# alebeck/jax-raft

Hardware: AMD Instinct MI355X
Metric: image-pairs/sec + Sintel-clean EPE, raft_large 32 iters at 1/2/4/8 MI355X (higher is better)
Workload: dtype bf16

## Files before the change

### csrc/kernels/conv_halo.hip

```cpp
#include "halo.h"

namespace {

template <int P>
JR_DEVICE constexpr int key_x(int key) { return P == 8 ? (key >> 1) & 7 : key & 15; }

JR_DEVICE int lane_px(int rho) {
  return rho < 4 ? rho : rho < 12 ? rho + 12 : rho < 16 ? rho - 8 : rho < 20 ? rho + 8 : rho < 28 ? rho - 12 : rho;
}

template <int CIN>
constexpr int pitch_of() { return CIN <= 64 ? 8 : CIN <= 128 ? 16 : 32; }

template <int CIN, int WCO, int WPX, int TN, bool INN>
constexpr int halo_min_blocks() {
  return TN > 2 ? 1 : CIN <= 64 ? 4 : CIN <= 96 ? (INN ? 3 : 1) : !INN ? 1 : WCO * WPX == 1 ? 4 : WCO * WPX <= 4 ? 2 : 1;
}

template <int CIN, int WCO, int WPX, int TN, int TR, int TC, bool INN, int KS = 3>
__global__ __launch_bounds__(64 * WCO * WPX, (halo_min_blocks<CIN, WCO, WPX, TN, INN>()))
void conv_halo_kernel(const ConvHaloParams p) {
  constexpr int NT = 64 * WCO * WPX;
  constexpr int P = pitch_of<CIN>();
  constexpr int CC = CIN / 8;
  constexpr int SPT = CIN / 16;
  constexpr int S = KS * KS * SPT;
  constexpr int PAD = KS / 2;
  constexpr bool WIDE = TN >= 4 && WCO * WPX > 4;
  constexpr bool MANY = WCO * WPX >= 12;
  constexpr int PD = S >= 16 ? (WCO * WPX >= 16 ? 4 : (WIDE || MANY || CIN <= 96) ? 8 : 16) : S;
  constexpr int FW = TC + KS - 1;
  constexpr int NFP = (TR + KS - 1) * FW;
  constexpr int RB = P * 16;
  static_assert(TR * TC <= 32 * WPX * TN && (TC == 16 || TC == 8), "tile");
  extern __shared__ __attribute__((aligned(16))) bf16 lds[];
  char* const lds_b = (char*)lds;
  const int tid = threadIdx.x, lane = tid & 63, wave = tid >> 6;
  const int rho = lane & 31, hh = lane >> 5;
  const int wc = wave % WCO, wp = wave / WCO;

  const int per_img = p.tiles_y * p.tiles_x;
  const int n = blockIdx.x / per_img;
  const int rem = blockIdx.x - n * per_img;
  const int ty = rem / p.tiles_x, tx = rem - ty * p.tiles_x;
  const int y0 = ty * TR, x0 = tx * TC;
// ... 284 lines not shown
```

### csrc/kernels/halo.h

```cpp
#pragma once
#include "conv_igemm.h"

namespace {

constexpr unsigned HOOB = 0x80000000u;
constexpr int FPITCH = 256;
constexpr int RPITCH = 128;

JR_DEVICE int f_off(int row, int chunk) { return row * FPITCH + (((chunk & 16) | ((chunk ^ row) & 15)) << 3); }
JR_DEVICE int r_off(int row, int chunk) { return row * RPITCH + (((chunk ^ row) & 15) << 3); }

JR_DEVICE u32x4 bload(__amdgpu_buffer_rsrc_t r, unsigned off) {
  return __builtin_bit_cast(u32x4, __builtin_amdgcn_raw_buffer_load_b128(r, off, 0, 0));
}

template <int NB, int S, int PD, typename LA, typename RB>
JR_DEVICE void pipe_gemm(f32x16 (&acc)[NB], bf16x8 (&ring)[PD], LA&& loadA, RB&& readB) {
#pragma unroll
  for (int b = 0; b < NB; ++b)
#pragma unroll
    for (int k = 0; k < 16; ++k) acc[b][k] = 0.f;
  bf16x8 bcur[NB], bnxt[NB];
#pragma unroll
  for (int b = 0; b < NB; ++b) bcur[b] = readB(0, b);
#pragma unroll
  for (int s = 0; s < S; ++s) {
    const bf16x8 a = ring[s % PD];
    if (s + PD < S) ring[s % PD] = loadA(s + PD);
    if (s + 1 < S) {
#pragma unroll
      for (int b = 0; b < NB; ++b) bnxt[b] = readB(s + 1, b);
    }
#pragma unroll
    for (int b = 0; b < NB; ++b) acc[b] = __builtin_amdgcn_mfma_f32_32x32x16_bf16(a, bcur[b], acc[b], 0, 0, 0);
#pragma unroll
    for (int b = 0; b < NB; ++b) bcur[b] = bnxt[b];
    __builtin_amdgcn_sched_group_barrier(0x100, NB, 0);
    __builtin_amdgcn_sched_group_barrier(0x020, 1, 0);
    __builtin_amdgcn_sched_group_barrier(0x008, NB, 0);
    asm volatile("" ::: "memory");
    __builtin_amdgcn_sched_barrier(0);
  }
}

}
```

### csrc/kernels/kernels.h

```cpp
#pragma once
#include <hip/hip_runtime.h>
#include <stdint.h>

extern "C" {

enum ConvEpi : int {
  EPI_STD = 0,
  EPI_GRU_A = 1,
  EPI_GRU_B = 2,
  EPI_BWD = 5,
  EPI_TAPS = 6,
};

struct BwdSeg {
  int mode;
  const void* gin; int gin_cs, gin_coff, gin_bf16;
  const void* mask; int mask_cs, mask_coff;
  int valid;
  void* out; int out_cs, out_coff, out_f32;
};

struct ConvParams {
  const void* x;
  int N, H, W;
// ... 149 lines not shown
int jr_unsup_loss_blocks(long P);
int jr_unsup_loss(const float* pred, const float* img1, const float* img2, const float* mask, const float* prm,
                  float* part, int B, int H, int W, int N, hipStream_t stream);
int jr_unsup_loss_bwd(const float* pred, const float* img1, const float* img2, const float* mask, const float* prm,
                      const float* scale, float* grad, int B, int H, int W, int N, hipStream_t stream);
long jr_census_tiles(int B, int H, int W);
int jr_census_gray(const float* img1, const float* img2, float* gray, int B, int H, int W, hipStream_t stream);
int jr_census_loss(const float* pred, const float* gray, const float* mask, const float* prm, float* part, float* coef,
                   int B, int H, int W, int N, hipStream_t stream);
int jr_census_loss_bwd(const float* pred, const float* gray, const float* coef, const float* scale, float* grad, int B,
                       int H, int W, int N, int add, hipStream_t stream);
#define JR_RANGE_MAX_PIXELS (1L << 23)
int jr_range_splat(const float* flow_fw, const float* flow_bw, int* acc, int B, int H, int W, hipStream_t stream);
int jr_range_visible(const float* flow_fw, const float* flow_bw, const int* acc, float* vis, int B, int H, int W,
                     int T, hipStream_t stream);
int jr_crop_resize(const float* x, const float* prm, float* out, int B, int H, int W, int C, int c, hipStream_t stream);
int jr_selfsup_loss_blocks(long P);
int jr_selfsup_loss(const float* pred, const float* target, const float* weight, const float* prm, float* part, int N,
                    int B, int H, int W, int Btot, int B0, hipStream_t stream);
int jr_selfsup_loss_bwd(const float* pred, const float* target, const float* weight, const float* prm, const float* scale,
                        float* grad, int N, int B, int H, int W, int Btot, int B0, hipStream_t stream);
struct Conv1x1Args {
  const void* x; int xcs, kvalid, kpad; const void* wpk; const float* bias; int act;
  void* y; int ycs, ycoff, cout, M;
};
int jr_flowin_dual(const void* x, int x_cstride, int N, int H, int W, int PH, int PW, const void* w,
                   const float* fbias, int cout, int relu, void* y, int y_cstride, int y_coff, int mode,
                   const void* feat, int feat_cstride, int feat_coff, const void* wpk, const float* cbias, float alpha,
                   const float* flow, float* out, const void* out_slot, long out_off, const Conv1x1Args* c1,
                   hipStream_t stream);
int jr_conv_direct(const void* x, int x_cstride, int N, int H, int W, int cin, int KH, int KW, int PH, int PW,
                   const void* w, const float* bias, int cout, int relu, void* y, int y_cstride, int y_coff,
                   hipStream_t stream);
int jr_copy_channels(const void* src, int s_cstride, int s_coff, void* dst, int d_cstride, int d_coff,
                     int M, int C, hipStream_t stream);

struct ConvF32Params {
  const float* x; int N, H, W, x_cs, x_coff, cin4;
  int KH, KW, SH, SW, PH, PW, OH, OW, M;
  const float* w; int K, cout;
  const float* bias; float alpha; int act, split;
  float* y; int y_cs, y_coff;
  float* y2; int y2_cs, y2_coff;
  const float* res; int res_cs, res_coff, res_post;
  float* h32; float* zbuf; int hidden;
  const float* bmap; int bmap_cs, bmap_coff;
  int ksplit; float* part;
};
int jr_conv_f32(const ConvF32Params* p, int epi, hipStream_t stream);
int jr_channel_stats_f32(const float* x, int N, int HW, int C, float* stats, float* partial, hipStream_t stream);
int jr_norm_act_f32(const float* x, const float* sx, int mode_x, const float* res, const float* sr, int mode_r,
                    float* y, int N, int HW, int C, float eps, int relu, hipStream_t stream);
int jr_prep_images_f32(const float* img1, const float* img2, int B, int H, int W, float* out, hipStream_t stream);
int jr_copy_channels_f32(const float* src, int s_cstride, int s_coff, float* dst, int d_cstride, int d_coff, int M,
                         int C, hipStream_t stream);
int jr_upsample_convex_f32(const float* mask, int mask_cstride, const float* flow, int B, int h, int w, float* out,
                           const void* out_slot, long out_off, hipStream_t stream);
int jr_corr_pool_f32(const float* src, long M, int hl, int wl, float* dst, hipStream_t stream);
int jr_corr_lookup_f32(const float* const* levels, int num_levels, int B, int h, int w, int nq, int radius,
                       const float* coords, float* out, int out_cstride, hipStream_t stream);
int jr_flow_update_f32(const float* delta, int dcs, int N, int h, int w, float* coords, float* flow32, float* hx,
                       int hx_cs, int hx_off, float* qx, int qx_cs, int qx_off, float* flow4, hipStream_t stream);

struct GruFusedParams {
  const void* hx; int hx_cs;
  const void* wa; const void* wb;
// ... 73 lines not shown
```

### csrc/runtime/binding.cpp

```cpp
#include <torch/custom_class.h>
#include <torch/library.h>
#include <ATen/ATen.h>
#include <c10/core/DeviceGuard.h>
#include <c10/hip/HIPStream.h>
#include <hip/hip_runtime.h>

#include <algorithm>
#include <array>
#include <functional>
#include <string>
#include <vector>

#include "../kernels/kernels.h"
#include "plan.h"

namespace jr {

using TList = c10::List<c10::optional<at::Tensor>>;
using IList = std::vector<int64_t>;

static inline at::Tensor opt(const TList& t, size_t i) {
  if (i >= t.size()) return at::Tensor();
  c10::optional<at::Tensor> v = t.get(i);
  return v.has_value() ? *v : at::Tensor();
// ... 787 lines not shown
              "taps_gemm: packed weights (pack_taps)");
  TORCH_CHECK(cs(taps) >= 24 && cs(taps) % 4 == 0 && taps.numel() >= M * cs(taps) &&
                  reinterpret_cast<uintptr_t>(taps.data_ptr()) % 16 == 0,
              "taps_gemm: taps [M][>=24], 16-byte rows");
  keep.push_back(fm); keep.push_back(wpk); keep.push_back(taps);
  const void* fp = fm.data_ptr();
  const void* wp = wpk.data_ptr();
  float* tp = taps.data_ptr<float>();
  const int fcs = cs(fm), tcs = cs(taps);
  return [=](hipStream_t s, int) { return jr_taps_gemm(fp, fcs, fcoff, K, wp, tp, tcs, (int)M, s); };
}

static Launch make_conv_direct(const TList& t, const IList& i, std::vector<at::Tensor>& keep) {
  at::Tensor x = opt(t, 0), w = opt(t, 1), bias = opt(t, 2), y = opt(t, 3);
  check_bf16(x, "x"); check_bf16(w, "w"); check_f32(bias, "bias"); check_bf16(y, "y");
  const int N = (int)i[0], H = (int)i[1], W = (int)i[2], cin = (int)i[3], KH = (int)i[4], KW = (int)i[5];
  const int PH = (int)i[6], PW = (int)i[7], cout = (int)i[8], relu = (int)i[9], y_coff = (int)i[10];
  const int64_t M = (int64_t)N * H * W;
  TORCH_CHECK(cs(x) >= cin && x.numel() >= M * cs(x), "conv_direct: x [N*H*W][>=cin]");
  const int kwp = KW <= 4 ? 4 : 8, nkc = (KH * kwp * 2 + 31) / 32;
  TORCH_CHECK(cin == 2 && w.numel() == (int64_t)cout * nkc * 32 && bias.numel() >= cout, "conv_direct: w / bias");
  TORCH_CHECK(y.numel() >= M * cs(y) && y_coff + cout <= cs(y), "conv_direct: y");
  for (auto& v : {x, w, bias, y}) keep.push_back(v);
  const void* xp = x.data_ptr();
  const void* wp = w.data_ptr();
  const float* bp = bias.data_ptr<float>();
  void* yp = y.data_ptr();
  const int xcs = cs(x), ycs = cs(y);
  return [=](hipStream_t s, int) {
    return jr_conv_direct(xp, xcs, N, H, W, cin, KH, KW, PH, PW, wp, bp, cout, relu, yp, ycs, y_coff, s);
  };
}

static Launch make_flowin_dual(const TList& t, const IList& i, double alpha, std::vector<at::Tensor>& keep) {
  Launch conv = make_conv_direct(t, IList(i.begin(), i.begin() + 11), keep);
  TORCH_CHECK((i.size() == 15 || i.size() == 21) && i[4] == 7 && i[5] == 7,
              "flowin_dual: expected 15 (+6) ints, a 7x7 flow conv");
  const bool has_c1 = i.size() == 21;
  Conv1x1Args c1a{};
  if (has_c1) {
    TORCH_CHECK(i[11] == 2 && i[17] == 352, "flowin_dual: the 1x1 conv part needs mode 2 and K padded to 352");
    TList t1;
    for (size_t k = 10; k < 14; ++k) t1.push_back(c10::optional<at::Tensor>(opt(t, k)));
    (void)make_conv1x1(t1, IList(i.begin() + 15, i.end()), keep);
    at::Tensor x1 = opt(t, 10), w1 = opt(t, 11), b1 = opt(t, 12), y1 = opt(t, 13);
    c1a = Conv1x1Args{x1.data_ptr(), (int)cs(x1), (int)i[16], (int)i[17], w1.data_ptr(), b1.data_ptr<float>(),
                      (int)i[19], y1.data_ptr(), (int)cs(y1), (int)i[20], (int)i[18], (int)i[15]};
  }
  at::Tensor x = opt(t, 0), w = opt(t, 1), bias = opt(t, 2), y = opt(t, 3), flow = opt(t, 4), out = opt(t, 5),
             slot = opt(t, 6), feat = opt(t, 7), wpk = opt(t, 8), cb = opt(t, 9);
  const int N = (int)i[0], H = (int)i[1], W = (int)i[2], PH = (int)i[6], PW = (int)i[7], cout = (int)i[8];
  const int relu = (int)i[9], y_coff = (int)i[10], mode = (int)i[11], fcoff = (int)i[14];
  const int64_t stride = i[12], slot_off = i[13];
  check_f32(flow, "flow32");
  TORCH_CHECK(mode == 1 || mode == 2, "flowin_dual: mode 1 (bilinear) or 2 (convex head)");
  TORCH_CHECK(flow.numel() >= (int64_t)N * H * W * 2, "flowin_dual: flow [M][2]");
  TORCH_CHECK(!slot.defined() || (slot.is_cuda() && slot.scalar_type() == at::kLong && slot.numel() == 1),
              "flowin_dual: out_slot must be one device int64");
  const int64_t cap = check_flow_out(out, N, H, W);
  TORCH_CHECK(stride >= 0 && stride % 8 == 0, "flowin_dual: iteration stride");
  int fcs = 0;
  if (mode == 2) {
    check_bf16(feat, "feat"); check_bf16(wpk, "wpk"); check_f32(cb, "cbias");
    fcs = cs(feat);
    TORCH_CHECK(fcs % 8 == 0 && fcoff % 8 == 0 && fcoff >= 0 && fcoff + 256 <= fcs &&
                    feat.numel() >= (int64_t)N * H * W * fcs && reinterpret_cast<uintptr_t>(feat.data_ptr()) % 16 == 0,
// ... 1332 lines not shown

static const std::vector<OpRow>& op_table() {
  static const std::vector<OpRow> rows = {
      row_tia("conv", "alpha", 22, 29, make_conv_fwd),
      row_tia("corr", "scale", 5, 7, make_corr),
      row_ti("lookup", 5, 9, make_lookup, 1),
      row_ti("feat_pool", 5, 5, make_feat_pool),
      row_ti("lookup_od", 6, 8, make_lookup_od, 1),
      row_ti("upsample_convex", 4, 4, make_upsample_convex),
      row_tia("convex_head", "alpha", 5, 7, make_convex_head),
      row_ti("upsample_bilinear", 4, 5, make_upsample_bilinear),
      row_ti("stats", 3, 3, make_stats),
      row_ti("stats_final", 3, 3, make_stats_final),
      row_tia("norm_act", "eps", 6, 6, make_norm_act),
      row_ti("prep", 3, 8, make_prep),
      row_ti("init_coords", 3, 3, make_init_coords),
      row_ti("init_flow", 5, 5, make_init_flow_bf16),
      row_ti("init_flow_f32", 5, 5, make_init_flow_f32),
      row_ti("forward_project", 4, 4, make_forward_project),
      row_ti("fb_check", 7, 9, make_fb_check),
      row_ti("warp_frames", 8, 10, make_warp_frames),
      row_t("memset", make_memset),
      row_t("copy", make_copy),
      row_ti("copy_channels", 4, 4, make_copy_channels),
      row_ti("sum_iters", 2, 2, make_sum_iters),
      row_ti("im2col", 11, 11, make_im2col),
      row_ti("flow_taps", 5, 5, make_flow_taps),
      row_ti("taps_gemm", 3, 3, make_taps_gemm),
      row_ti("gru_fused", 4, 5, make_gru_fused),
      row_ti("gru_fused_me", 4, 4, make_gru_fused_me),
      row_ti("gru_halo", 9, 9, make_gru_halo),
      row_ti("conv1x1", 6, 6, make_conv1x1),
      row_ti("conv_direct", 11, 11, make_conv_direct),
      row_tia("flowin_dual", "alpha", 15, 21, make_flowin_dual),
      row_tia("upsample_convex_bwd", "alpha", 3, 3, make_upsample_convex_bwd),
      row_ti("upsample_bilinear_bwd", 3, 3, make_upsample_bilinear_bwd),
      row_ti("flow_gather_bwd", 3, 3, make_flow_gather_bwd),
      row_ti("lookup_bwd", 5, 6, make_lookup_bwd),
      row_tia("norm_bwd", "eps", 5, 5, make_norm_bwd),
      row_ti("pack", 2, 2, make_pack),
      row_ti("wgrad", 16, 16, make_wgrad),
      row_ti("bn_table", 2, 2, make_bn_table),
      row_ti("augment_sums", 3, 3, make_augment_sums_of<JR_AUGMENT_DENSE>),
      row_ti("augment", 5, 5, make_augment_gather_of<JR_AUGMENT_DENSE>),
      row_ti("augment_sparse_sums", 3, 3, make_augment_sums_of<JR_AUGMENT_SPARSE>),
      row_ti("augment_sparse", 5, 5, make_augment_gather_of<JR_AUGMENT_SPARSE>),
      row_ti("augment_mixed_sums", 2, 2, make_augment_sums_of<JR_AUGMENT_MIXED>),
      row_ti("augment_mixed", 4, 4, make_augment_gather_of<JR_AUGMENT_MIXED>),
      row_ti("flow_metrics", 6, 6, make_flow_metrics),
      row_ti("unsup_loss", 4, 4, make_unsup_loss),
      row_ti("unsup_loss_bwd", 4, 4, make_unsup_loss_bwd),
      row_ti("census_gray", 3, 3, make_census_gray),
      row_ti("census_loss", 4, 4, make_census_loss),
      row_ti("census_loss_bwd", 5, 5, make_census_loss_bwd),
      row_ti("range_splat", 3, 3, make_range_splat),
      row_ti("range_visible", 4, 4, make_range_visible),
      row_ti("crop_resize", 5, 5, make_crop_resize),
      row_ti("selfsup_loss", 6, 6, make_selfsup_loss),
      row_ti("selfsup_loss_bwd", 6, 6, make_selfsup_loss_bwd),
      row_tia("conv_f32", "alpha", 22, 22, make_conv_f32),
      row_ti("stats_f32", 3, 3, make_stats_f32),
      row_tia("norm_act_f32", "eps", 6, 6, make_norm_act_f32),
      row_ti("prep_f32", 3, 3, make_prep_f32),
      row_ti("copy_channels_f32", 4, 4, make_copy_channels_f32),
      row_ti("upsample_convex_f32", 4, 5, make_upsample_convex_f32),
      row_ti("corr_pool_f32", 3, 3, make_corr_pool_f32),
// ... 108 lines not shown
```

### jax_raft_amd/_build.py

```python
from __future__ import annotations

import concurrent.futures as cf
import os
import subprocess
import sys
import sysconfig
from pathlib import Path

PKG_DIR = Path(__file__).resolve().parent
REPO = PKG_DIR.parent
CSRC = REPO / "csrc"
BUILD = REPO / "build" / "native"
SO_PATH = PKG_DIR / "_C.so"
ARCH = os.environ.get("JR_OFFLOAD_ARCH") or "gfx950"
HIPCC = os.environ.get("HIPCC", "/opt/rocm/bin/hipcc")
CXX = os.environ.get("CXX", "g++")

KERNEL_SOURCES = [
    CSRC / "kernels" / "conv_igemm.hip",
    CSRC / "kernels" / "conv_fam_r.hip",
    CSRC / "kernels" / "conv_fam_rw.hip",
    CSRC / "kernels" / "conv_fam_p.hip",
    CSRC / "kernels" / "conv_fam_m32.hip",
    CSRC / "kernels" / "conv_fam_d2.hip",
    CSRC / "kernels" / "conv_fam_g.hip",
    CSRC / "kernels" / "corr.hip",
    CSRC / "kernels" / "corr_pyr.hip",
    CSRC / "kernels" / "corr_od.hip",
    CSRC / "kernels" / "elementwise.hip",
    CSRC / "kernels" / "conv_f32.hip",
    CSRC / "kernels" / "f32.hip",
    CSRC / "kernels" / "flowhead.hip",
    CSRC / "kernels" / "conv_direct.hip",
    CSRC / "kernels" / "train.hip",
    CSRC / "kernels" / "wgrad.hip",
    CSRC / "kernels" / "convex_head.hip",
    CSRC / "kernels" / "conv1x1.hip",
    CSRC / "kernels" / "gru_fused.hip",
    CSRC / "kernels" / "gru_halo.hip",
    CSRC / "kernels" / "conv_halo.hip",
    CSRC / "kernels" / "bgemm.hip",
    CSRC / "kernels" / "merged.hip",
    CSRC / "kernels" / "conv_fam_grp.hip",
    CSRC / "kernels" / "warm.hip",
    CSRC / "kernels" / "fbcheck.hip",
    CSRC / "kernels" / "framewarp.hip",
    CSRC / "kernels" / "augment.hip",
    CSRC / "kernels" / "metrics.hip",
    CSRC / "kernels" / "unsup.hip",
    CSRC / "kernels" / "census.hip",
    CSRC / "kernels" / "occlusion.hip",
    CSRC / "kernels" / "selfsup.hip",
]
HOST_SOURCES = [CSRC / "runtime" / "binding.cpp", CSRC / "runtime" / "png.cpp"]
HEADERS = sorted(CSRC.rglob("*.h"))


def _torch_paths():
    import torch
    from torch.utils import cpp_extension

    inc = cpp_extension.include_paths(device_type="cuda")
    lib = os.path.join(os.path.dirname(torch.__file__), "lib")
    abi = int(torch._C._GLIBCXX_USE_CXX11_ABI)
    return inc, lib, abi

# ... 70 lines not shown
```

### jax_raft_amd/ops/native.py

```python
from __future__ import annotations

import math
import threading
from dataclasses import dataclass
from pathlib import Path
from typing import List, Optional, Sequence, Tuple

import torch

from .. import knobs
from .._build import SO_PATH as _DEFAULT_SO

SO_PATH = Path(knobs.get("JR_NATIVE_SO")).resolve() if knobs.get("JR_NATIVE_SO") else _DEFAULT_SO

_lock = threading.Lock()
_loaded = False
_load_error: Optional[BaseException] = None

ACT_NONE, ACT_RELU, ACT_SIGMOID, ACT_TANH, ACT_SPLIT_TANH_RELU = 0, 1, 2, 3, 4
EPI_STD, EPI_GRU_A, EPI_GRU_B = 0, 1, 2
EPI_BWD, EPI_TAPS = 5, 6
TAPS_CFGS = (34, 22, 35, 38)
CFG_TILES = {0: (128, 128), 1: (64, 128), 2: (128, 64), 3: (16, 256), 4: (64, 64), 5: (16, 64)}
CFG_TILES.update({6: (128, 128), 7: (64, 128), 8: (128, 64), 9: (128, 256), 10: (64, 64), 11: (256, 128)})
CFG_TILES.update({12: (128, 128), 13: (64, 128), 14: (128, 64), 15: (64, 64)})
CFG_TILES.update({16: (256, 128), 17: (128, 256)})
CFG_TILES.update({18: (128, 128), 19: (128, 128), 20: (256, 128)})
CFG_TILES.update({21: (128, 128), 22: (256, 128), 23: (128, 64), 24: (64, 128)})
CFG_TILES.update({25: (256, 128), 26: (128, 256), 27: (128, 128), 28: (64, 256)})
CFG_TILES.update({33: (128, 128), 34: (256, 128)})
CFG_TILES.update({35: (256, 128), 36: (128, 128), 37: (128, 128), 38: (256, 128), 39: (256, 128), 40: (128, 256),
                  41: (64, 128), 42: (256, 128), 43: (256, 128)})
TUNE_CFGS = (0, 1, 2, 3, 4, 5, 12, 13, 14, 15, 18, 19, 20, 21, 22, 23, 24, 25, 26, 27, 28, 33, 34,
             35, 38)
NUM_CUS = 256
GROUPED_CFGS = frozenset((2, 4, 5, 23, 24, 12, 14, 15))


def gru_fused_tiles(N: int, H: int, W: int, vertical: int) -> int:
    if not vertical:
        return N * H if 1 <= W <= 128 else 0
    J = 2 if 2 * H <= 128 and W % 2 == 0 else 1
    return N * (W // J) if 1 <= H and J * H <= 128 and J * (H + 4) <= 136 and W % J == 0 else 0


def _m32_chan(r: torch.Tensor) -> torch.Tensor:
    return 16 * ((r >> 2) & 1) + (r & 3) + 4 * (r >> 3)


def pack_gru_halo(kernel: torch.Tensor, cin_pad: int, out: Optional[torch.Tensor] = None) -> torch.Tensor:
    kh, kw, cin, cout = kernel.shape
    assert cout % 32 == 0 and cin <= cin_pad and cin_pad % 16 == 0, (kernel.shape, cin_pad)
    dev = kernel.device
    k = torch.zeros(kh * kw, cin_pad, cout, dtype=torch.float32, device=dev)
    k[:, :cin] = kernel.detach().float().reshape(kh * kw, cin, cout)
    k = k.reshape(kh * kw * cin_pad, cout)
    ks = kh * kw * cin_pad // 16
    blk = torch.arange(cout // 32, device=dev).view(-1, 1, 1, 1)
    s = torch.arange(ks, device=dev).view(1, -1, 1, 1)
    l = torch.arange(64, device=dev).view(1, 1, 64, 1)
    j = torch.arange(8, device=dev).view(1, 1, 1, 8)
    kk = (16 * s + 8 * (l >> 5) + j).expand(cout // 32, ks, 64, 8)
    co = (32 * blk + _m32_chan(l & 31)).expand(cout // 32, ks, 64, 8)
    w = k[kk, co].to(torch.bfloat16).contiguous()
    if out is not None:
        assert out.shape == w.shape and out.dtype == torch.bfloat16
        out.copy_(w)
        return out
    return w


GRU_HALO_BLOCKS = {(128, 0): ((1, 1), (2, 1), (2, 2), (3, 2), (3, 3), (5, 4)), (96, 1): ((2, 1), (2, 2), (3, 2))}


def gru_halo_lds(hd: int, mode: int, TR: int, TC: int, nb1: int, nb2: int) -> int:
    f_rows = TC + 8 if mode == 0 else (TR + 4) * (TC + 4)
# ... 305 lines not shown
    lane = torch.arange(64, device=dev).view(1, 1, 1, 64, 1)
    j = torch.arange(8, device=dev).view(1, 1, 1, 1, 8)
    o = 16 * t + lane % 16
    c = 64 * g + 16 * (lane // 16) + 8 * s + j
    return wt[o.expand(4, 2, 2, 64, 8), c.expand(4, 2, 2, 64, 8)].to(torch.bfloat16).contiguous()


CONV1X1_KPADS = (128, 256, 352, 384)


def pack_conv1x1(kernel: torch.Tensor, kpad: int) -> torch.Tensor:
    _, _, K, N = kernel.shape
    assert N % 64 == 0 and K <= kpad and kpad % 32 == 0, (kernel.shape, kpad)
    w = torch.zeros(kpad, N, dtype=torch.float32, device=kernel.device)
    w[:K] = kernel.detach().float().reshape(K, N)
    dev = kernel.device
    g, ks, t, l, j = torch.meshgrid(torch.arange(N // 64, device=dev), torch.arange(kpad // 32, device=dev),
                                    torch.arange(4, device=dev), torch.arange(64, device=dev),
                                    torch.arange(8, device=dev), indexing="ij")
    r = l & 15
    k = 32 * ks + 8 * (l >> 4) + j
    co = 64 * g + 16 * (r >> 2) + 4 * t + (r & 3)
    return w[k, co].to(torch.bfloat16).reshape(-1).contiguous()


def conv1x1(x: torch.Tensor, wpk: torch.Tensor, bias: torch.Tensor, kvalid: int, kpad: int, cout: int,
            act: int = ACT_NONE) -> torch.Tensor:
    M = x.shape[0]
    y = torch.empty(M, cout, device=x.device, dtype=torch.bfloat16)
    ops().conv1x1([x, wpk, bias, y], [M, kvalid, kpad, cout, act, 0])
    return y


def pack_taps(kernel: torch.Tensor) -> torch.Tensor:
    kh, kw, K, co = kernel.shape
    assert (kh, kw, co) == (3, 3, 2) and K % 32 == 0, kernel.shape
    w = kernel.detach().float().reshape(9, K, 2).permute(1, 0, 2).reshape(K, 18)
    a = torch.zeros(K, 32, dtype=torch.float32, device=kernel.device)
    a[:, :18] = w
    a = a.reshape(K // 32, 4, 8, 2, 16)
    return a.permute(0, 3, 1, 4, 2).contiguous().to(torch.bfloat16).reshape(-1)


def taps_gemm(fm: torch.Tensor, wpk: torch.Tensor, K: int, coff: int = 0) -> torch.Tensor:
    M = fm.shape[0]
    out = torch.empty(M, 24, device=fm.device, dtype=torch.float32)
    ops().taps_gemm([fm, wpk, out], [M, K, coff])
    return out


def convex_head(feat: torch.Tensor, wpk: torch.Tensor, bias: torch.Tensor, flow: torch.Tensor, B: int, h: int,
                w: int, alpha: float, coff: int = 0, out: Optional[torch.Tensor] = None, tiles: int = 0) -> torch.Tensor:
    if out is None:
        out = torch.empty(B, 8 * h, 8 * w, 2, device=feat.device, dtype=torch.float32)
    ops().convex_head([feat, wpk, bias, flow, out], [B, h, w, coff, 0, tiles], float(alpha))
    return out


def project_keys(B: int, h: int, w: int, device) -> torch.Tensor:
    return torch.full((2 * B * h * w + 2,), -1, dtype=torch.int64, device=device)


def forward_project(flow: torch.Tensor, fill_radius: int = 4, keys: Optional[torch.Tensor] = None,
                    out: Optional[torch.Tensor] = None) -> torch.Tensor:
    if not flow.is_cuda:
        from ..models.reference import forward_project as golden
# ... 591 lines not shown
```

### jax_raft_amd/runtime/engine.py

```python
from __future__ import annotations

import itertools
import operator
import weakref
from collections import OrderedDict
from dataclasses import dataclass, field
from typing import Dict, List, Optional, Tuple

import torch

from ..models.reference import BidirectionalFlow, BidirectionalWarp
from ..models.layers import (
    NORM_BATCH,
    NORM_CUSTOM,
    NORM_INSTANCE,
    BottleneckBlock,
    ConvNormActivation,
    CorrBlock,
    FeatureEncoder,
    FlowHead,
    MaskPredictor,
    MotionEncoder,
    RecurrentBlock,
    ResidualBlock,
# ... 91 lines not shown
    pw = (((W0 // 8) + 1) * 8 - W0) % 8
    return ph // 2, ph - ph // 2, pw // 2, pw - pw // 2


_U8_LUT: Dict[str, torch.Tensor] = {}


def u8_table(device) -> torch.Tensor:
    key = str(device)
    t = _U8_LUT.get(key)
    if t is None:
        t = _U8_LUT[key] = (torch.arange(256, dtype=torch.float32) / 255.0 * 2.0 - 1.0).to(device)
    return t


class RaftEngine:

    def __new__(cls, *args, precision: str = "bf16", **kwargs):
        if precision not in ("bf16", "fp32", "mixed"):
            raise ValueError(f"precision must be 'bf16', 'fp32' or 'mixed', got {precision!r}")
        if precision == "fp32" and cls is RaftEngine:
            from .engine_f32 import RaftEngineF32
            cls = RaftEngineF32
        elif precision == "mixed" and cls is RaftEngine:
            from .engine_f32 import RaftEngineMixed
            cls = RaftEngineMixed
        return super().__new__(cls)

    precision = "bf16"
    fe_external = False

    GRU = "auto"
    GRU_ME = "auto"
    PRO_LANES = "auto"
    HALO_NORM = True
    MERGED_UP = True
    CONV_GROUP = True
    MASK_PARITY = False
    CORR_PERSIST_B1 = True
    HOST_GATE = True
    WARM_FILL_RADIUS = 4

    def __init__(self, model, device, use_graph: bool = True, copy_output: bool = True,
                 corr_dtype: torch.dtype = torch.bfloat16, gate_dtype: torch.dtype = torch.bfloat16,
                 autotune: bool = True, streams="auto", split: int = 1,
                 cfg_override: Optional[Dict[str, int]] = None, cp_group=None, **mode):
        mode.pop("precision", None)
        corr = mode.pop("corr", "volume")
        if mode:
            raise TypeError(f"RaftEngine: unexpected keyword arguments {sorted(mode)}")
        if corr not in ("volume", "on_demand"):
            raise ValueError(f"corr must be 'volume' or 'on_demand', got {corr!r}")
        if corr == "on_demand":
            if self.precision != "bf16":
                raise NotImplementedError(f"corr='on_demand': not with precision={self.precision!r} (the on-demand "
                                          "lookup is lowered for the bf16 engine only)")
            if cp_group is not None:
                raise NotImplementedError("corr='on_demand': not with context parallelism (cp_group splits the "
                                          "volume the on-demand path never builds)")
        self.corr_mode = corr
        nat.require()
        self._init_cp(cp_group)
        assert streams in (True, False, "auto"), streams
        self.streams_mode = streams
        self.halo_norm = bool(self.HALO_NORM)
        self.halo_res = self.halo_norm
# ... 655 lines not shown
                    nat.ops().gru_halo(t, base + list(tile))
                e_.record()
                e_.synchronize()
                el = s_.elapsed_time(e_)
                if best is None or el < best[0]:
                    best = (el, c)
            code = best[1]
            tunedb.record(self.arch, key, code)
        code = self._agree(code)
        _TUNE_CACHE[key + (str(self.device),)] = code
        self.chosen_cfgs[f"gru{gi}.halo"] = code
        return enc[code]

    def _gru_fused_ok(self, B: int, h: int, w: int) -> bool:
        env = "1" if self.GRU == "fused" else "auto"
        rb = self.model.update_block.recurrent_block
        ks = [tuple(k) for k in rb.kernel_size]
        if (self.hidden != 128 or self.hx_cs != 256 or self.gate_cs < 384 or ks != [(1, 5), (5, 1)]
                or self.gate_dtype != torch.bfloat16):
            return False
        tiles = min(nat.gru_fused_tiles(B, h, w, 0), nat.gru_fused_tiles(B, h, w, 1))
        return tiles > 0 and (env == "1" or tiles >= 3 * nat.NUM_CUS // 4)

    def _gru_me_ok(self, B: int, h: int, w: int) -> bool:
        assert self.GRU_ME in ("auto", "on", "off"), self.GRU_ME
        if self.GRU_ME == "off" or self.cp:
            return False
        sp = self._specs["me.conv"]
        ks = tuple(self.model.update_block.recurrent_block.kernel_size[0])
        if (not (sp.halo_ks == 3 and sp.cin8 == 256 and sp.cout <= 128 and self.mot_off == 128 and self.hx_cs == 256)
                or ks != (1, 5) or not 1 <= w <= 128):
            return False
        return self.GRU_ME == "on" or nat.gru_fused_tiles(B, h, w, 0) >= 3 * nat.NUM_CUS // 4

    def _parts(self, B: int) -> int:
        return self.split if (self.split > 1 and B % self.split == 0 and not self.cp) else 1

    def uses_lanes(self, B: int, all_iters: bool = True, *, parts: Optional[int] = None) -> bool:
        if self.cp or not self._lanes_ok(all_iters):
            return False
        if self.streams_mode != "auto":
            return bool(self.streams_mode)
        return B // (self._parts(B) if parts is None else parts) >= self.AUTO_STREAMS_MIN_BATCH

    def _build(self, B: int, H: int, W: int, n_iters: int, all_iters: bool = True,
               src: Optional[Tuple[int, int, int, int]] = None, warm: bool = False, *,
               parts: Optional[int] = None, slot: bool = False) -> _PlanState:
        return lowering.build(self, B, H, W, n_iters, all_iters, src, warm, parts=parts, slot=slot)

    def _build_bidir(self, B: int, H: int, W: int, n_iters: int, all_iters: bool,
                     src: Optional[Tuple[int, int, int, int]], warp: bool = False, *, slot: bool = False) -> _PlanState:
        return lowering.build_bidir(self, B, H, W, n_iters, all_iters, src, warp, slot=slot)

    @torch.no_grad()
    def forward(self, image1: torch.Tensor, image2: torch.Tensor, num_flow_updates: int = 12,
                return_all_iters: bool = True, flow_init=None, return_flow_low: bool = False,
                bidirectional: bool = False, fb_alpha: float = 0.01, fb_beta: float = 0.5, warp: bool = False):
        if self._stale():
            self._pack()
            self._last = None
        if self.cp and flow_init is not None:
            raise NotImplementedError("forward(flow_init=...): not with context parallelism (cp_group)")
        if warp and not bidirectional:
            raise ValueError("forward(warp=True) requires bidirectional=True (the warp is the last op of the "
                             "bidirectional plan)")
        if bidirectional and self.corr_mode == "on_demand":
# ... 221 lines not shown
```

### jax_raft_amd/runtime/lowering.py

```python
from __future__ import annotations

from dataclasses import dataclass
from typing import Optional, Tuple

import torch

from ..ops import native as nat
from ..ops.native import ACT_RELU, ACT_SPLIT_TANH_RELU, EPI_GRU_A, EPI_GRU_B, EPI_TAPS, round_up
from . import engine as _engine

BF16, F32 = torch.bfloat16, torch.float32

E_PREP, E_CTX, E_FLOW, E_FH, E_MASK, E_FE2 = range(6)


@dataclass(frozen=True)
class PartChoices:
    schedule: str
    all_iters: bool
    warm: bool
    bidir: bool
    lanes: Tuple[int, int, int]
    lanes_on: bool
    pro_on: bool
    pro_lanes: Tuple[int, int, int]
    fe_split: bool
    s2d: bool
    blocked: int
    bl: int
    on_demand: bool
    split_mask: bool
    s1: str
    taps_epi: bool
    gru_path: str
    gru_me: bool
    halo_pp: bool
    qx_x: bool
    hm: bool
    parity: bool
    mask_wait: Optional[int]
    merged_up: bool
    c1_merged: bool


def _prologue_choices(eng, Bi: int, h: int, w: int, lanes, slot: bool) -> dict:
    main, side, _ = lanes
    lanes_on = main != side
    pl = eng.PRO_LANES
    assert pl in ("auto", "on", "off"), pl
    pro_on = pl == "on" or (pl == "auto" and Bi * h * w <= 4 * 55 * 128)
    pro_lanes = tuple(lanes) if lanes_on or eng.cp or not pro_on else (main, 1, 2)
    fe_split = pro_lanes[0] != pro_lanes[1] and not (pl == "auto" and Bi == 1)
    blocked = int(eng.corr_dtype == BF16 and w % 16 == 0 and (h * w) % 8 == 0 and not eng.cp)
    bl = 2 if (blocked and eng.CORR_PERSIST_B1 and not slot) else blocked
    return dict(lanes=tuple(lanes), lanes_on=lanes_on, pro_on=pro_on, pro_lanes=pro_lanes, fe_split=fe_split,
                s2d="fe.stem_s2d" in eng._specs and "ce.stem_s2d" in eng._specs,
                blocked=blocked, bl=bl, on_demand=eng.corr_mode == "on_demand")


def _gru_choices(eng, B: int, h: int, w: int, lanes_on: bool) -> dict:
    ngru = len(eng.model.update_block.recurrent_block.kernel_size)
    gru_path = eng._gru_path(B, h, w)
    if gru_path == "fused" and eng.cp:
        gru_path = "unfused"
    halo_pp = gru_path == "halo" and ngru == 1
    hm = gru_path != "unfused" and eng.has_mask and (lanes_on or halo_pp)
    parity = bool(hm and gru_path == "fused" and eng._convex_w is not None and eng.MASK_PARITY)
    mask_wait = None if not lanes_on or parity else ngru - 1 if (gru_path == "halo" or hm) else 0
    return dict(gru_path=gru_path, halo_pp=halo_pp, hm=hm, parity=parity, mask_wait=mask_wait,
                gru_me=gru_path == "fused" and eng._gru_me_ok(B, h, w), qx_x=gru_path != "halo" or halo_pp)


def _head_choices(eng, B: int, all_iters: bool, lanes_on: bool) -> dict:
    sp = eng._specs
    me = eng.model.update_block.motion_encoder
    split_mask = lanes_on or eng.cp
    s1 = "fh1.flow" if eng.has_mask and not (all_iters and not split_mask) else "fh1"
    taps_epi = eng._taps_epi_w is not None and sp[s1].cout == 256
    flow7 = eng._cf1_w is not None and tuple(me.convflow1.layers_0.kernel.shape[:2]) == (7, 7)
    merged_up = bool(flow7 and not eng.cp and (not eng.has_mask or (eng._convex_w is not None and not taps_epi))
                     and eng.MERGED_UP)
    c1_merged = (merged_up and eng.has_mask and len(me.corr_layers) == 2 and eng._cc1_w is not None
                 and eng._cc1_kpad == 352)
    schedule = ("cp" if eng.cp else "lanes" if lanes_on else "one_lane" if all_iters
                else "final_merged" if flow7 and B < eng.AUTO_STREAMS_MIN_BATCH else "final")
    return dict(split_mask=split_mask, s1=s1, taps_epi=taps_epi, merged_up=merged_up, c1_merged=c1_merged,
                schedule=schedule)


def choose(eng, Bi: int, B: int, h: int, w: int, all_iters: bool, lanes, *, warm: bool = False,
           bidir: bool = False, slot: bool = False) -> PartChoices:
    assert not (bidir and (warm or eng.cp)), "bidirectional plans: one part, cold, no context parallelism"
    pro = _prologue_choices(eng, Bi, h, w, lanes, slot)
    assert not (pro["on_demand"] and (bidir or eng.cp)), "on-demand plans: one direction, no context parallelism"
    gru, head = _gru_choices(eng, B, h, w, pro["lanes_on"]), _head_choices(eng, B, all_iters, pro["lanes_on"])
    return PartChoices(all_iters=bool(all_iters), warm=warm, bidir=bidir, **pro, **gru, **head)


class PartRecorder:

    def __init__(self, eng, st, plan, c: PartChoices, b0: int, Bi: int, H: int, W: int, pt: str):
        self.eng, self.st, self.plan, self.c, self.pt = eng, st, plan, c, pt
        self.b0, self.Bi, self.B = b0, Bi, 2 * Bi if c.bidir else Bi
        self.H, self.W, self.h, self.w = H, W, H // 8, W // 8
        self.M, self.L = self.B * self.h * self.w, eng.num_levels
        ub = eng.model.update_block
        self.me, self.ngru = ub.motion_encoder, len(ub.recurrent_block.kernel_size)
        self.inp1, self.inp2 = st.inp1[b0:b0 + Bi], st.inp2[b0:b0 + Bi]
        self.out = st.out[:, b0:b0 + self.B]
        self.out_off = (self.out.data_ptr() - st.out.data_ptr()) // 4
        self.stride = st.out.shape[1] * H * W * 2

    def alloc(self, name, shape, dtype=BF16):
        t = self.st.bufs[self.pt + name] = torch.zeros(shape, dtype=dtype, device=self.eng.device)
        return t

    def record(self):
        for step in (self.state_buffers, self.prep, self.context, self.features, self.correlation, self.loop_buffers,
                     getattr(self, "schedule_" + self.c.schedule)):
            step()
        self.plan.set_lane(0)
        self.plan.set_segment(2)

    def state_buffers(self):
        e, p, M = self.eng, self.plan, self.M
        p.set_segment(0)
        p.set_lane(self.c.pro_lanes[0])
        self.hx, self.qx = self.alloc("hx", (M, e.hx_cs)), self.alloc("qx", (M, e.hx_cs))
# ... 60 lines not shown

    def correlation(self):
        e, p, c, Bi, B, h, w, L = self.eng, self.plan, self.c, self.Bi, self.B, self.h, self.w, self.L
        fmap, pad = self.fmap, [None] * (4 - L)
        self.slabs = e._cp_slabs(h) if e.cp else [(0, h)]
        self.r0, self.r1 = r0, r1 = self.slabs[e.cp_rank]
        self.nq = nq = (r1 - r0) * w
        self.pooled = ([self.alloc(f"fpool.l{l}", (Bi, h >> l, w >> l, e.fmap_ch), F32) for l in range(1, L)]
                       if c.on_demand else [])
        self.levels = levels = []
        for l in range(0 if c.on_demand else L):
            shape = ((self.M, -(-h // 8) * (8 >> l), -(-w // 16) * (16 >> l)) if c.blocked and l < 2
                     else (B * nq, h >> l, w >> l))
            levels.append(self.alloc(f"corr.l{l}", shape, e.corr_dtype))
        scale = 1.0 / float(e.fmap_ch) ** 0.5
        if c.on_demand:
            p.add_feat_pool([fmap[Bi:]] + self.pooled, [Bi, h, w, e.fmap_ch, L])
        elif e.cp:
            for b in range(B):
                p.add_corr([fmap[b, r0:r1], fmap[B + b]] + [v[b * nq:(b + 1) * nq] for v in levels] + pad,
                           [1, h, w, e.fmap_ch, L, nq, 0], scale)
        else:
            p.add_corr([fmap[:Bi], fmap[Bi:]] + levels + pad, [Bi, h, w, e.fmap_ch, L, h * w, c.bl], scale)
            if c.bidir:
                p.add_corr([fmap[Bi:], fmap[:Bi]] + [v[Bi * h * w:] for v in levels] + pad,
                           [Bi, h, w, e.fmap_ch, L, h * w, c.bl], scale)
        p.add_wait(E_CTX)

    def loop_buffers(self):
        e, c, M = self.eng, self.c, self.M
        cl, fl = self.me.corr_layers, self.me.flow_layers
        self.corr = self.alloc("corr", (M, e.corr_cs))
        self.cf = self.alloc("cf", (M, cl[-1] + fl[-1]))
        self.f1 = self.alloc("f1", (M, fl[0]))
        self.c1 = self.alloc("c1", (M, cl[0])) if len(cl) == 2 else None
        self.taps = self.alloc("fh2.taps", (M, 24), F32)
        self.fm = None if c.taps_epi else self.alloc("fm", (M, round_up(e._specs[c.s1].cout, 8)))
        self.mfeat = (self.alloc("mfeat", (M, round_up(e._specs["mask.convrelu"].cout, 8)))
                      if e.has_mask and (c.split_mask or not c.all_iters) else None)
        self.mask = self.alloc("mask", (M, 576)) if e.has_mask and e._convex_w is None else None
        self.hm = self.alloc("hm", (M, e.hidden)) if c.hm else None
        self.hm2 = self.alloc("hm2", (M, e.hidden)) if c.parity else None
        self.flow32b = self.alloc("flow32b", (M, 2), F32) if c.parity else None
        self.st.flow_out.append((self.b0, self.B, self.flow32, self.flow32b))

    def flow_features(self):
        e, p, B, h, w = self.eng, self.plan, self.B, self.h, self.w
        if e._cf1_w is not None:
            p.add_conv_direct([self.flow8, e._cf1_w, e._cf1_b, self.f1], self._flowin_ints())
        else:
            e._conv(p, e._specs["me.convflow1"], self.flow8, B, h, w, self.f1, act=ACT_RELU)
        e._conv(p, e._specs["me.convflow2"], self.f1, B, h, w, self.cf, y_coff=self.me.corr_layers[-1], act=ACT_RELU)

    def _flowin_ints(self):
        c = self.me.convflow1.layers_0
        kh, kw_, _, co = c.kernel.shape
        return [self.B, self.h, self.w, 2, kh, kw_, c.padding[0], c.padding[1], co, 1, 0]

    def flowin_dual(self, stride: int, convex: bool):
        e, cl = self.eng, self.me.corr_layers
        t_ = [self.flow8, e._cf1_w, e._cf1_b, self.f1, self.flow32, self.out, self.st.out_slot]
        if not convex:
            self.plan.add_flowin_dual(t_, self._flowin_ints() + [1, stride, self.out_off, 0], 1.0)
            return
        t_ += [self.fm, e._convex_w, e._convex_b]
        i_ = self._flowin_ints() + [2, stride, self.out_off, e.fh_hidden]
        if self.c.c1_merged:
            t_ += [self.corr, e._cc1_w, e._cc1_b, self.c1]
            i_ += [self.M, e.corr_cs, e._cc1_kpad, cl[0], ACT_RELU, 0]
        self.plan.add_flowin_dual(t_, i_, e.model.mask_predictor.multiplier)

    def flow_head(self):
        e, p, c, B, h, w = self.eng, self.plan, self.c, self.B, self.h, self.w
        s1 = e._specs[c.s1]
        if c.taps_epi:
            e._conv(p, s1, self.hx, B, h, w, self.taps, act=ACT_RELU, epi=EPI_TAPS, tapw=e._taps_epi_w)
            return
        if c.halo_pp:
            e._conv(p, s1, self.qx, B, h, w, self.fm, x_alt=self.hx, act=ACT_RELU)
        else:
# ... 279 lines not shown
```

Measured before the change: 419.2.

## Fuse convflow1 7x7 and convflow2 3x3 into one tiled kernel

```diff
diff --git a/csrc/kernels/conv_halo.hip b/csrc/kernels/conv_halo.hip
--- a/csrc/kernels/conv_halo.hip
+++ b/csrc/kernels/conv_halo.hip
@@ -1,16 +1,6 @@
 #include "halo.h"
 
 namespace {
-
-template <int P>
-JR_DEVICE constexpr int key_x(int key) { return P == 8 ? (key >> 1) & 7 : key & 15; }
-
-JR_DEVICE int lane_px(int rho) {
-  return rho < 4 ? rho : rho < 12 ? rho + 12 : rho < 16 ? rho - 8 : rho < 20 ? rho + 8 : rho < 28 ? rho - 12 : rho;
-}
-
-template <int CIN>
-constexpr int pitch_of() { return CIN <= 64 ? 8 : CIN <= 128 ? 16 : 32; }
 
 template <int CIN, int WCO, int WPX, int TN, bool INN>
 constexpr int halo_min_blocks() {
diff --git a/csrc/kernels/flowfeat.hip b/csrc/kernels/flowfeat.hip
--- /dev/null
+++ b/csrc/kernels/flowfeat.hip
@@ -0,0 +1,142 @@
+#include "halo.h"
+
+namespace {
+
+constexpr int C1 = 128, COUT = 64;
+constexpr int WCO = 2, WPX = 2, TN = 2, TR = 8, TC = 16;
+constexpr int NT = 64 * WCO * WPX;
+constexpr int P = pitch_of<C1>();
+constexpr int SPT = C1 / 16, S = 9 * SPT, PD = 16;
+constexpr int FW = TC + 2, FH = TR + 2, NFP = FH * FW;
+constexpr int RB = P * 16;
+constexpr int KH = 7, KWP = 8, NKC = 4, PAD7 = 3;
+constexpr int PR = FH + KH, PC = FW + KWP - 1;
+constexpr int PATCH_OFF = NFP * RB;
+constexpr int LDS_BYTES = PATCH_OFF + (PR * PC * 4 + 15) / 16 * 16;
+constexpr int NPT = (NFP + 15) / 16;
+static_assert(NT % 64 == 0 && NT / 64 * 32 == C1, "one 32-channel block of convflow1 per wave");
+static_assert(TR * TC == 32 * WPX * TN && COUT == 32 * WCO, "tile");
+
+__global__ __launch_bounds__(NT, 1) void flow_features_kernel(const FlowFeatParams p) {
+  extern __shared__ __attribute__((aligned(16))) bf16 lds[];
+  char* const lds_b = (char*)lds;
+  unsigned* const patch = (unsigned*)(lds_b + PATCH_OFF);
+  const int tid = threadIdx.x, lane = tid & 63, wave = tid >> 6;
+  const int rho = lane & 31, hh = lane >> 5;
+  const int wc = wave % WCO, wp = wave / WCO;
+
+  const int per_img = p.tiles_y * p.tiles_x;
+  const int n = blockIdx.x / per_img;
+  const int rem = blockIdx.x - n * per_img;
+  const int ty = rem / p.tiles_x, tx = rem - ty * p.tiles_x;
+  const int y0 = ty * TR, x0 = tx * TC;
+
+  const __amdgpu_buffer_rsrc_t ws = __builtin_amdgcn_make_buffer_rsrc((void*)p.w2, (short)0, (int)p.w2_bytes, 0x00020000);
+  const unsigned w_base = (unsigned)(wc * S * 64 + lane) * 16u;
+  bf16x8 ring[PD];
+#pragma unroll
+  for (int d = 0; d < PD; ++d) ring[d] = __builtin_bit_cast(bf16x8, bload(ws, w_base + (unsigned)d * 1024u));
+
+  {
+    const unsigned* fl = (const unsigned*)p.flow + (long)n * p.H * p.W;
+    for (int e = tid; e < PR * PC; e += NT) {
+      const int pr = e / PC, pc = e - pr * PC;
+      const int iy = y0 - 1 - PAD7 + pr, ix = x0 - 1 - PAD7 + pc;
+      const bool in = (unsigned)iy < (unsigned)p.H && (unsigned)ix < (unsigned)p.W;
+      patch[e] = in ? fl[iy * p.W + ix] : 0u;
+    }
+  }
+  const int li = lane & 15, kg = lane >> 4;
+  const int co0 = wave * 32;
+  bf16x8 a[2][NKC];
+  float bv1[2][4];
+#pragma unroll
+  for (int t = 0; t < 2; ++t) {
+#pragma unroll
+    for (int kc = 0; kc < NKC; ++kc) a[t][kc] = ((const bf16x8*)p.w1)[((co0 / 16 + t) * NKC + kc) * 64 + lane];
+#pragma unroll
+    for (int r = 0; r < 4; ++r) bv1[t][r] = p.b1[co0 + 16 * t + 4 * kg + r];
+  }
+  __syncthreads();
+#pragma unroll 4
+  for (int pt = 0; pt < NPT; ++pt) {
+    const int f = pt * 16 + li;
+    const bool live = f < NFP;
+    const int ff = live ? f : 0;
+    const int fy = ff / FW, fx = ff - fy * FW;
+    u32x4 u[NKC];
+#pragma unroll
+    for (int kc = 0; kc < NKC; ++kc) {
+      const int tt0 = kc * 16 + 4 * kg;
+      const unsigned* q = patch + (fy + tt0 / KWP) * PC + fx + tt0 % KWP;
+#pragma unroll
+      for (int e = 0; e < 4; ++e) u[kc][e] = q[e];
+    }
+    f32x4 acc[2] = {f32x4{0.f, 0.f, 0.f, 0.f}, f32x4{0.f, 0.f, 0.f, 0.f}};
+#pragma unroll
+    for (int kc = 0; kc < NKC; ++kc) {
+      const bf16x8 b = __builtin_bit_cast(bf16x8, u[kc]);
+#pragma unroll
+      for (int t = 0; t < 2; ++t) acc[t] = __builtin_amdgcn_mfma_f32_16x16x32_bf16(a[t][kc], b, acc[t], 0, 0, 0);
+    }
+    if (!live) continue;
+    const bool in = (unsigned)(y0 - 1 + fy) < (unsigned)p.H && (unsigned)(x0 - 1 + fx) < (unsigned)p.W;
+    const int kx = key_x<P>(fx + TC * fy);
+#pragma unroll
+    for (int t = 0; t < 2; ++t) {
+      bf16x4 o;
+#pragma unroll
+      for (int r = 0; r < 4; ++r) o[r] = f2bf(in ? fmaxf(acc[t][r] + bv1[t][r], 0.f) : 0.f);
+      *(bf16x4*)(lds_b + ff * RB + (((4 * wave + 2 * t + (kg >> 1)) ^ kx) << 4) + 8 * (kg & 1)) = o;
+    }
+  }
+
+  int rb0[TN], key0[TN], om[TN];
+#pragma unroll
+  for (int b = 0; b < TN; ++b) {
+    const int q = 32 * (wp * TN + b) + lane_px(rho);
+    const int i = q / TC, j = q - i * TC;
+    const bool ok = i < TR && y0 + i < p.H && x0 + j < p.W;
+    rb0[b] = ok ? (i * FW + j) * RB : 0;
+    key0[b] = ok ? j + TC * i : 0;
+    om[b] = ok ? (n * p.H + y0 + i) * p.W + x0 + j : -1;
+  }
+  __syncthreads();
+
+  f32x16 acc[TN];
+  pipe_gemm<TN, S, PD>(
+      acc, ring,
+      [&](int s) { return __builtin_bit_cast(bf16x8, bload(ws, w_base + (unsigned)s * 1024u)); },
+      [&](int s, int b) {
+        const int tap = s / SPT, kc = s - tap * SPT;
+        const int u = tap / 3, v = tap % 3;
+        const int kxh = (key_x<P>(key0[b] + v + TC * u) ^ hh) << 4;
+        return *(const bf16x8*)(lds_b + (rb0[b] + (((2 * kc) << 4) ^ kxh)) + (u * FW + v) * RB);
+      });
+  const int c0 = 32 * wc + 16 * hh;
+  float bv[16];
+#pragma unroll
+  for (int k = 0; k < 16; ++k) bv[k] = p.b2[c0 + k];
+#pragma unroll
+  for (int b = 0; b < TN; ++b) {
+    const int m = om[b];
+    if (m < 0) continue;
+    float v[16];
+#pragma unroll
+    for (int k = 0; k < 16; ++k) v[k] = fmaxf(acc[b][k] + bv[k], 0.f);
+    store_bf16<16>((bf16*)p.y + (long)m * p.ycs + p.yoff + c0, v);
+  }
+}
+
+}
+
+extern "C" int jr_flow_features_tile(int* out2) {
+  out2[0] = TR; out2[1] = TC;
+  return LDS_BYTES;
+}
+
+extern "C" int jr_flow_features_fused(const FlowFeatParams* p, hipStream_t stream) {
+  if (p->ntiles <= 0 || p->ycs % 8 != 0 || p->yoff % 8 != 0 || p->yoff + COUT > p->ycs) return (int)hipErrorInvalidValue;
+  hipLaunchKernelGGL(flow_features_kernel, dim3(p->ntiles), dim3(NT), LDS_BYTES, stream, *p);
+  return (int)hipGetLastError();
+}
diff --git a/csrc/kernels/halo.h b/csrc/kernels/halo.h
--- a/csrc/kernels/halo.h
+++ b/csrc/kernels/halo.h
@@ -13,6 +13,16 @@
 JR_DEVICE u32x4 bload(__amdgpu_buffer_rsrc_t r, unsigned off) {
   return __builtin_bit_cast(u32x4, __builtin_amdgcn_raw_buffer_load_b128(r, off, 0, 0));
 }
+
+template <int P>
+JR_DEVICE constexpr int key_x(int key) { return P == 8 ? (key >> 1) & 7 : key & 15; }
+
+JR_DEVICE int lane_px(int rho) {
+  return rho < 4 ? rho : rho < 12 ? rho + 12 : rho < 16 ? rho - 8 : rho < 20 ? rho + 8 : rho < 28 ? rho - 12 : rho;
+}
+
+template <int CIN>
+constexpr int pitch_of() { return CIN <= 64 ? 8 : CIN <= 128 ? 16 : 32; }
 
 template <int NB, int S, int PD, typename LA, typename RB>
 JR_DEVICE void pipe_gemm(f32x16 (&acc)[NB], bf16x8 (&ring)[PD], LA&& loadA, RB&& readB) {
diff --git a/csrc/kernels/kernels.h b/csrc/kernels/kernels.h
--- a/csrc/kernels/kernels.h
+++ b/csrc/kernels/kernels.h
@@ -205,6 +205,15 @@
 int jr_conv_direct(const void* x, int x_cstride, int N, int H, int W, int cin, int KH, int KW, int PH, int PW,
                    const void* w, const float* bias, int cout, int relu, void* y, int y_cstride, int y_coff,
                    hipStream_t stream);
+struct FlowFeatParams {
+  const void* flow; int N, H, W;
+  const void* w1; const float* b1;
+  const void* w2; long w2_bytes; const float* b2;
+  void* y; int ycs, yoff;
+  int tiles_y, tiles_x, ntiles;
+};
+int jr_flow_features_fused(const FlowFeatParams* p, hipStream_t stream);
+int jr_flow_features_tile(int* out2);
 int jr_copy_channels(const void* src, int s_cstride, int s_coff, void* dst, int d_cstride, int d_coff,
                      int M, int C, hipStream_t stream);
 
diff --git a/csrc/runtime/binding.cpp b/csrc/runtime/binding.cpp
--- a/csrc/runtime/binding.cpp
+++ b/csrc/runtime/binding.cpp
@@ -843,6 +843,35 @@
   };
 }
 
+static Launch make_flow_features_fused(const TList& t, const IList& i, std::vector<at::Tensor>& keep) {
+  at::Tensor x = opt(t, 0), w1 = opt(t, 1), b1 = opt(t, 2), w2 = opt(t, 3), b2 = opt(t, 4), y = opt(t, 5);
+  check_bf16(x, "flow"); check_bf16(w1, "w1"); check_f32(b1, "b1"); check_bf16(w2, "w2"); check_f32(b2, "b2");
+  check_bf16(y, "y");
+  const int N = (int)i[0], H = (int)i[1], W = (int)i[2], y_coff = (int)i[3];
+  TORCH_CHECK(N > 0 && H > 0 && W > 0, "flow_features_fused: N, H, W");
+  const int64_t M = (int64_t)N * H * W;
+  TORCH_CHECK(M < (1LL << 31) / 256, "flow_features_fused: too many pixels");
+  TORCH_CHECK(cs(x) == 2 && x.numel() == M * 2, "flow_features_fused: compact 2-channel flow [N*H*W][2]");
+  TORCH_CHECK(w1.numel() == 128 * 4 * 32 && b1.numel() == 128, "flow_features_fused: 7x7 conv 2 -> 128 (pack_direct_weight)");
+  TORCH_CHECK(w2.numel() == 64 * 9 * 128 && b2.numel() == 64, "flow_features_fused: 3x3 conv 128 -> 64 (pack_halo_conv)");
+  TORCH_CHECK(cs(y) % 8 == 0 && y_coff % 8 == 0 && y_coff >= 0 && y_coff + 64 <= cs(y) && y.numel() >= M * cs(y),
+              "flow_features_fused: y");
+  for (const at::Tensor* v : {&w1, &w2, &y})
+    TORCH_CHECK(reinterpret_cast<uintptr_t>(v->data_ptr()) % 16 == 0, "flow_features_fused: 16-byte aligned operands");
+  TORCH_CHECK(reinterpret_cast<uintptr_t>(x.data_ptr()) % 4 == 0, "flow_features_fused: 4-byte aligned flow");
+  int tile[2];
+  jr_flow_features_tile(tile);
+  FlowFeatParams p{};
+  p.flow = x.data_ptr(); p.N = N; p.H = H; p.W = W;
+  p.w1 = w1.data_ptr(); p.b1 = b1.data_ptr<float>();
+  p.w2 = w2.data_ptr(); p.w2_bytes = (long)w2.numel() * 2; p.b2 = b2.data_ptr<float>();
+  p.y = y.data_ptr(); p.ycs = cs(y); p.yoff = y_coff;
+  p.tiles_y = (H + tile[0] - 1) / tile[0]; p.tiles_x = (W + tile[1] - 1) / tile[1];
+  p.ntiles = N * p.tiles_y * p.tiles_x;
+  for (auto& v : {x, w1, b1, w2, b2, y}) keep.push_back(v);
+  return [p](hipStream_t s, int) { return jr_flow_features_fused(&p, s); };
+}
+
 static Launch make_flowin_dual(const TList& t, const IList& i, double alpha, std::vector<at::Tensor>& keep) {
   Launch conv = make_conv_direct(t, IList(i.begin(), i.begin() + 11), keep);
   TORCH_CHECK((i.size() == 15 || i.size() == 21) && i[4] == 7 && i[5] == 7,
@@ -2241,6 +2270,7 @@
       row_ti("gru_halo", 9, 9, make_gru_halo),
       row_ti("conv1x1", 6, 6, make_conv1x1),
       row_ti("conv_direct", 11, 11, make_conv_direct),
+      row_ti("flow_features_fused", 4, 4, make_flow_features_fused),
       row_tia("flowin_dual", "alpha", 15, 21, make_flowin_dual),
       row_tia("upsample_convex_bwd", "alpha", 3, 3, make_upsample_convex_bwd),
       row_ti("upsample_bilinear_bwd", 3, 3, make_upsample_bilinear_bwd),
diff --git a/jax_raft_amd/_build.py b/jax_raft_amd/_build.py
--- a/jax_raft_amd/_build.py
+++ b/jax_raft_amd/_build.py
@@ -32,6 +32,7 @@
     CSRC / "kernels" / "f32.hip",
     CSRC / "kernels" / "flowhead.hip",
     CSRC / "kernels" / "conv_direct.hip",
+    CSRC / "kernels" / "flowfeat.hip",
     CSRC / "kernels" / "train.hip",
     CSRC / "kernels" / "wgrad.hip",
     CSRC / "kernels" / "convex_head.hip",
diff --git a/jax_raft_amd/ops/native.py b/jax_raft_amd/ops/native.py
--- a/jax_raft_amd/ops/native.py
+++ b/jax_raft_amd/ops/native.py
@@ -42,6 +42,10 @@
         return N * H if 1 <= W <= 128 else 0
     J = 2 if 2 * H <= 128 and W % 2 == 0 else 1
     return N * (W // J) if 1 <= H and J * H <= 128 and J * (H + 4) <= 136 and W % J == 0 else 0
+
+
+def flow_fused_tiles(N: int, H: int, W: int) -> int:
+    return N * -(-H // 8) * -(-W // 16)
 
 
 def _m32_chan(r: torch.Tensor) -> torch.Tensor:
@@ -413,6 +417,16 @@
     return y
 
 
+def flow_features_fused(flow: torch.Tensor, w1: torch.Tensor, b1: torch.Tensor, spec2: ConvSpec, N: int, H: int,
+                        W: int, y: torch.Tensor, y_coff: int = 0) -> torch.Tensor:
+    assert flow.dtype == torch.bfloat16 and flow.shape[-1] == 2 and flow.numel() == N * H * W * 2 and flow.is_contiguous()
+    assert w1.numel() == 128 * 4 * 32 and b1.numel() == 128, "7x7 conv 2 -> 128 (pack_direct_weight)"
+    assert spec2.halo_ks == 3 and spec2.cin8 == 128 and spec2.cout == 64 and spec2.wh is not None, "3x3 conv 128 -> 64"
+    assert y.dtype == torch.bfloat16 and y.shape[-1] % 8 == 0 and y_coff % 8 == 0 and y_coff + 64 <= y.shape[-1]
+    ops().flow_features_fused([flow, w1, b1, spec2.wh, spec2.b, y], [N, H, W, y_coff])
+    return y
+
+
 def pack_taps(kernel: torch.Tensor) -> torch.Tensor:
     kh, kw, K, co = kernel.shape
     assert (kh, kw, co) == (3, 3, 2) and K % 32 == 0, kernel.shape
diff --git a/jax_raft_amd/runtime/engine.py b/jax_raft_amd/runtime/engine.py
--- a/jax_raft_amd/runtime/engine.py
+++ b/jax_raft_amd/runtime/engine.py
@@ -147,6 +147,7 @@
 
     GRU = "auto"
     GRU_ME = "auto"
+    FLOW_FUSED = "auto"
     PRO_LANES = "auto"
     HALO_NORM = True
     MERGED_UP = True
@@ -868,6 +869,17 @@
                 or ks != (1, 5) or not 1 <= w <= 128):
             return False
         return self.GRU_ME == "on" or nat.gru_fused_tiles(B, h, w, 0) >= 3 * nat.NUM_CUS // 4
+
+    def _flow_fused_ok(self, B: int, h: int, w: int, lanes_on: bool) -> bool:
+        assert self.FLOW_FUSED in ("auto", "on", "off"), self.FLOW_FUSED
+        if self.FLOW_FUSED == "off" or not lanes_on or self.cp or self.precision != "bf16" or self._cf1_w is None:
+            return False
+        me = self.model.update_block.motion_encoder
+        c1, sp = me.convflow1.layers_0, self._specs["me.convflow2"]
+        if (tuple(c1.kernel.shape) != (7, 7, 2, 128) or tuple(c1.padding) != (3, 3)
+                or not (sp.halo_ks == 3 and sp.cin8 == 128 and sp.cout == 64 and sp.wh is not None)):
+            return False
+        return self.FLOW_FUSED == "on" or nat.flow_fused_tiles(B, h, w) >= 3 * nat.NUM_CUS // 4
 
     def _parts(self, B: int) -> int:
         return self.split if (self.split > 1 and B % self.split == 0 and not self.cp) else 1
diff --git a/jax_raft_amd/runtime/lowering.py b/jax_raft_amd/runtime/lowering.py
--- a/jax_raft_amd/runtime/lowering.py
+++ b/jax_raft_amd/runtime/lowering.py
@@ -41,6 +41,7 @@
     mask_wait: Optional[int]
     merged_up: bool
     c1_merged: bool
+    flow_fused: bool
 
 
 def _prologue_choices(eng, Bi: int, h: int, w: int, lanes, slot: bool) -> dict:
@@ -71,7 +72,7 @@
                 gru_me=gru_path == "fused" and eng._gru_me_ok(B, h, w), qx_x=gru_path != "halo" or halo_pp)
 
 
-def _head_choices(eng, B: int, all_iters: bool, lanes_on: bool) -> dict:
+def _head_choices(eng, B: int, h: int, w: int, all_iters: bool, lanes_on: bool) -> dict:
     sp = eng._specs
     me = eng.model.update_block.motion_encoder
     split_mask = lanes_on or eng.cp
@@ -84,8 +85,9 @@
                  and eng._cc1_kpad == 352)
     schedule = ("cp" if eng.cp else "lanes" if lanes_on else "one_lane" if all_iters
                 else "final_merged" if flow7 and B < eng.AUTO_STREAMS_MIN_BATCH else "final")
+    flow_fused = schedule == "lanes" and eng._flow_fused_ok(B, h, w, lanes_on)
     return dict(split_mask=split_mask, s1=s1, taps_epi=taps_epi, merged_up=merged_up, c1_merged=c1_merged,
-                schedule=schedule)
+                schedule=schedule, flow_fused=flow_fused)
 
 
 def choose(eng, Bi: int, B: int, h: int, w: int, all_iters: bool, lanes, *, warm: bool = False,
@@ -93,7 +95,7 @@
     assert not (bidir and (warm or eng.cp)), "bidirectional plans: one part, cold, no context parallelism"
     pro = _prologue_choices(eng, Bi, h, w, lanes, slot)
     assert not (pro["on_demand"] and (bidir or eng.cp)), "on-demand plans: one direction, no context parallelism"
-    gru, head = _gru_choices(eng, B, h, w, pro["lanes_on"]), _head_choices(eng, B, all_iters, pro["lanes_on"])
+    gru, head = _gru_choices(eng, B, h, w, pro["lanes_on"]), _head_choices(eng, B, h, w, all_iters, pro["lanes_on"])
     return PartChoices(all_iters=bool(all_iters), warm=warm, bidir=bidir, **pro, **gru, **head)
 
 
@@ -220,7 +222,7 @@
         cl, fl = self.me.corr_layers, self.me.flow_layers
         self.corr = self.alloc("corr", (M, e.corr_cs))
         self.cf = self.alloc("cf", (M, cl[-1] + fl[-1]))
-        self.f1 = self.alloc("f1", (M, fl[0]))
+        self.f1 = None if c.flow_fused else self.alloc("f1", (M, fl[0]))
         self.c1 = self.alloc("c1", (M, cl[0])) if len(cl) == 2 else None
         self.taps = self.alloc("fh2.taps", (M, 24), F32)
         self.fm = None if c.taps_epi else self.alloc("fm", (M, round_up(e._specs[c.s1].cout, 8)))
@@ -234,6 +236,11 @@
 
     def flow_features(self):
         e, p, B, h, w = self.eng, self.plan, self.B, self.h, self.w
+        if self.c.flow_fused:
+            sp2 = e._specs["me.convflow2"]
+            p.add_flow_features_fused([self.flow8, e._cf1_w, e._cf1_b, sp2.wh, sp2.b, self.cf],
+                                      [B, h, w, self.me.corr_layers[-1]])
+            return
         if e._cf1_w is not None:
             p.add_conv_direct([self.flow8, e._cf1_w, e._cf1_b, self.f1], self._flowin_ints())
         else:
```

Result: faster. 432.8, median of 6 (+3.3%).
